# jeremy29tien/robosuite-benchmark

Hardware: AMD Instinct MI355X
Metric: SAC grad-steps/sec (batch=256, 1e6 buffer) at 1/2/4/8 GPU (higher is better)
Workload: dtype f32; 1 GPU; Lift-Panda-OSC-POSE SAC inner loop: obs 42 / act 7, batch 256, 1000000-slot HBM replay buffer (full), hidden 256x256, variant.json trainer_kwargs (lr 1e-3/5e-4, tau .005, period 5); parallelism=single GPU

## Files before the change

### robosuite_benchmark_amd/csrc/sac_fused.h

```cpp
#pragma once

constexpr int CNT_STRIDE = 32;
constexpr unsigned long long HANDOFF_TIMEOUT_TICKS = 5000000ull;

template <int SLEEP = 1>
__device__ __forceinline__ int handoff_wait(const unsigned *cnt, unsigned target, unsigned *abort_flag) {
    const unsigned long long t0 = __builtin_amdgcn_s_memrealtime();
    for (;;) {
        const unsigned v = __hip_atomic_load(cnt, __ATOMIC_RELAXED, __HIP_MEMORY_SCOPE_AGENT);
        if ((int)(v - target) >= 0) return 1;
        if (__hip_atomic_load(abort_flag, __ATOMIC_RELAXED, __HIP_MEMORY_SCOPE_AGENT) != 0u) return 0;
        if (__builtin_amdgcn_s_memrealtime() - t0 > HANDOFF_TIMEOUT_TICKS) {
            __hip_atomic_store(abort_flag, 1u, __ATOMIC_RELAXED, __HIP_MEMORY_SCOPE_AGENT);
            return 0;
        }
        __builtin_amdgcn_s_sleep(SLEEP);
    }
}

template <int SLEEP = 1>
__device__ __forceinline__ void handoff_wait_multi(int n, const unsigned *c0, unsigned t0, const unsigned *c1, unsigned t1,
                                                   const unsigned *c2, unsigned t2, unsigned *abort_flag, int *s_ok) {
    if (threadIdx.x < 64) {
        const int l = threadIdx.x;
// ... 45 lines not shown
__device__ __forceinline__ unsigned long long multi_lp_peek(int n, const unsigned *c0, const unsigned *c1, const unsigned long long *lp_tag, int NB) {
    unsigned long long w = 0ull;
    if (threadIdx.x < 64) {
        const int l = threadIdx.x;
        if (l < n) w = __hip_atomic_load(l == 0 ? c0 : c1, __ATOMIC_RELAXED, __HIP_MEMORY_SCOPE_AGENT);
        else if (l >= 16 && l < 16 + NB) w = __hip_atomic_load(lp_tag + (l - 16), __ATOMIC_RELAXED, __HIP_MEMORY_SCOPE_AGENT);
    }
    return w;
}

__device__ __forceinline__ void handoff_publish(unsigned *cnt) {
    asm volatile("s_waitcnt vmcnt(0) lgkmcnt(0)\n\ts_barrier" ::: "memory");
    if (threadIdx.x == 0) __hip_atomic_fetch_add(cnt, 1u, __ATOMIC_RELAXED, __HIP_MEMORY_SCOPE_AGENT);
}

__device__ __forceinline__ AlphaStep alpha_step_v(const Ctl *ctl, const float *part_logpi, int NB, int B, float target_entropy,
                                                  float lr, int auto_alpha, double bc1, double bc2s) {
    AlphaStep r;
    const float la = sload(&ctl->log_alpha), m0 = sload(&ctl->a_m), v0 = sload(&ctl->a_v);
    if (!auto_alpha) { r.alpha = 1.0f; r.alpha_loss = 0.0f; r.log_alpha = la; r.m = m0; r.v = v0; return r; }
    const int lane = threadIdx.x & 63;
    const float mine = part_logpi[lane < NB ? lane : 0];
    float sum = 0.f;
#pragma unroll
    for (int i = 0; i < 16; ++i)
        if (i < NB) sum += __builtin_bit_cast(float, __builtin_amdgcn_readlane(__builtin_bit_cast(int, mine), i));
    const float mean_lp = sum / (float)B + target_entropy;
    r.alpha_loss = -((la * mean_lp) + 0.0f);
    const float gr = -mean_lp;
    r.m = m0 + ADAM_1MB1 * (gr - m0);
    r.v = v0 * ADAM_B2 + ADAM_1MB2 * gr * gr;
    const float step_size = (float)((double)lr / bc1);
    const float denom = sqrtf(r.v) / (float)bc2s + 1e-8f;
    r.log_alpha = la + (-step_size * r.m) / denom;
    r.alpha = expf(r.log_alpha);
    return r;
}

template <int D>
__device__ __forceinline__ bool split_first_layer(WRing<1, D> &rq, const float *X0, int KLQ, int KS, float bq, float *zx_blk,
                                                  unsigned *cnt, unsigned target, unsigned *abort_flag, int *s_ok, int part,
                                                  f32x4 (&z)[4]) {
    const int wave = threadIdx.x >> 6, lane = threadIdx.x & 63;
    f32x4 acc[1] = {};
    gemm_ring<false, false>(rq, X0, KLQ, KS, acc);
    f32x4 zq;
#pragma unroll
    for (int i = 0; i < 4; ++i) zq[i] = acc[0][i] + bq;
    st4_sc1(zx_blk + ((part * 4 + wave) * 64 + lane) * 4, zq);
    handoff_publish(cnt);
    if (threadIdx.x == 0) *s_ok = handoff_wait(cnt, target, abort_flag);
    lds_barrier();
    if (!*s_ok) return false;
#pragma unroll
    for (int t = 0; t < 4; ++t) z[t] = ld4(zx_blk + ((wave * 4 + t) * 64 + lane) * 4);
    return true;
}

template <int PAGES>
struct ImgRegs {
    f32x4 v[PAGES];
    __device__ __forceinline__ void issue(const float *__restrict__ img, int KL) {
        const float *p = img + (threadIdx.x >> 4) * KL + 4 * (threadIdx.x & 15);
#pragma unroll
        for (int j = 0; j < PAGES; ++j) {
            v[j] = f32x4{0.f, 0.f, 0.f, 0.f};
            if (64 * j < KL) v[j] = ld4(p + 64 * j);
        }
    }
    __device__ __forceinline__ void commit(float *X, int KL, int skip_k = -1) const {
        const int row = threadIdx.x >> 4, c = threadIdx.x & 15;
        float *p = X + row * KL + 4 * c;
        const int sp = (skip_k >= 0 && ((c ^ row) >> 2) == ((skip_k >> 4) & 3)) ? (skip_k >> 6) : -1;
#pragma unroll
        for (int j = 0; j < PAGES; ++j)
            if (64 * j < KL && j != sp) st4(p + 64 * j, v[j]);
    }
};

template <int NTH, bool WIDE, int MODE = M_SAC, bool IMG = false>
__global__ __launch_bounds__(256) void k_abc(Dev d, const float *__restrict__ S, SlotLayout SL, StepArg sa) {
    kernarg_prefetch<sizeof(Dev) + 8 + sizeof(SlotLayout) + sizeof(StepArg)>();
    constexpr int SP = 4, SW = 64;
    extern __shared__ __attribute__((aligned(16))) float lds[];
    __shared__ int s_ok;
    __shared__ float s_dq[RB];
    __shared__ float s_lp[16];
    const int B = d.B, O = d.O, A = d.A, NB = d.NB;
    const int KLQ = (d.KQ + 63) & ~63;
    float *X0 = lds;
    float *X1 = X0 + RB * KLQ;
    float *XS = X1 + RB * H;
    float *red = XS + RB * SW;
    float *WL = red + FUSED_RED;
#ifndef SAC_XR_XOR
#define SAC_XR_XOR 4
#endif
    const int xq = blockIdx.x >> 3, xr = (blockIdx.x & 7) ^ SAC_XR_XOR;
    const bool isq = xr < 4;
    const int net = (xr >> 1) & 1;
    const int bi = 2 * xq + (xr & 1);
    const int part = bi & 3, rb = bi >> 2;
    const int row0 = rb * RB;
    const int wave = threadIdx.x >> 6, lane = threadIdx.x & 63, c = lane & 15, g = lane >> 4;
    const int row = threadIdx.x >> 4, a = threadIdx.x & 15, grow = row0 + row;
    const int n0 = SW * part + 16 * wave;
    unsigned *cnt_head = d.cnt, *cnt_qa = d.cnt + (size_t)2 * NB * CNT_STRIDE, *cnt_tq = d.cnt + (size_t)3 * NB * CNT_STRIDE,
             *cnt_ac = d.cnt + (size_t)4 * NB * CNT_STRIDE;
    unsigned *cnt_zx = d.cnt + (size_t)(5 * NB + 2) * CNT_STRIDE;
    unsigned long long *lp_tag = reinterpret_cast<unsigned long long *>(d.cnt + (size_t)(11 * NB + 2) * CNT_STRIDE);
    const unsigned seq = sa.seq;
    const bool own_s = isq && net == 0 && part == 0, own_n = !isq && net == 0 && part == 0;
    if ((sa.pad2 & 1u) && blockIdx.x == (4 ^ SAC_XR_XOR)) return;
    STAMP(0, 0);
    float eps = 0.f;
    f32x4 keep1[4], zkeep[4];
    float bv1[1], w3[4];
    unsigned peek = 0u;
    const bool skip_a = (MODE == M_TD3_CRITIC) && !isq && net == 0 && !(sa.pad2 & 4u);
    if (!skip_a) {
        const float *P = isq ? d.P[1 + net] : ((MODE == M_TD3_CRITIC && net == 1) ? d.P[5] : d.P[0]);
        const Layer L0 = isq ? d.LQ[0] : d.LP[0], L1 = isq ? d.LQ[1] : d.LP[1], L2 = isq ? d.LQ[2] : d.LP[2];
        const int K0 = isq ? d.KQ : d.KP;
        const float *obs = S + ((!isq && net) ? SL.off_nobs : SL.off_obs) + (size_t)row0 * O;
        RowRegs<IMG ? 1 : (WIDE ? 32 : 8)> rows;
        ImgRegs<IMG ? (WIDE ? 8 : 2) : 1> img;
        if constexpr (IMG) img.issue(S + ((!isq && net) ? SL.off_img_n : SL.off_img_sa) + (size_t)row0 * KLQ, KLQ);
        else rows.issue(K0, obs, O, O, S + SL.off_act + (size_t)row0 * A, isq ? A : 0, A, d.KP);
        WRing<4, WIDE ? 1 : RD0> r0;
        WRing<1, 8> rq;
        constexpr int PRE0 = 2;
        float bv0[4], bq = 0.f;
        if constexpr (WIDE) {
            rq.init(P + L0.offW, L0.Kp, 64 * part + 16 * wave, 16);
            rq.fill(K0 >> 4);
            bq = P[L0.offB + 64 * part + 16 * wave + c];
        } else {
            r0.init(P + L0.offW, L0.Kp, 64 * wave, 16);
            r0.fill_part(K0 >> 4, 0, PRE0);
#pragma unroll
            for (int t = 0; t < 4; ++t) bv0[t] = P[L0.offB + 64 * wave + 16 * t + c];
        }
        SB();
        WRing<1, 8> r1;
        r1.init(P + L1.offW, H, n0, 16);
        if constexpr (WIDE) r1.fill(H >> 4);
        WRing<NTH, 1> rh;
#define ABC_LATE_REQUESTS()                                                                             \
        do {                                                                                            \
            bv1[0] = P[L1.offB + n0 + c];                                                               \
            _Pragma("unroll") for (int u = 0; u < 4; ++u) w3[u] = 0.f;                                  \
            if (!isq) {                                                                                 \
                rh.init(P + L2.offW, H, 0, 16, 4 * part + wave);                                        \
                rh.fill(1);                                                                             \
            } else {                                                                                    \
                _Pragma("unroll") for (int u = 0; u < 4; ++u) w3[u] = P[L2.offW + frag_off(0, SW * part + a + 16 * u, H)]; \
            }                                                                                           \
            SB();                                                                                       \
        } while (0)
        if constexpr (WIDE) ABC_LATE_REQUESTS();
        STAMP(0, 12);
        {
            const int side0 = isq ? 0 : 1;
            const float *epp0 = side0 ? d.eps2 : d.eps1;
            if (a < A && !epp0) eps = philox_normal(d.noise_seed, (unsigned long long)sa.step_now, (unsigned)(grow * 16 + a), side0 ? 1u : 0u);
        }
        if constexpr (IMG) img.commit(X0, KLQ);
        else rows.commit(X0, KLQ, K0, O, d.KP, isq ? A : 0);
        lds_barrier();
        STAMP(0, 13);
        if constexpr (WIDE) {
            const int chain = isq ? net : 2 + net;
            if (!split_first_layer(rq, X0, KLQ, K0 >> 4, bq, d.zx + (size_t)(chain * NB + rb) * (RB * H),
                                   cnt_zx + (size_t)(chain * NB + rb) * CNT_STRIDE, 4u * seq, d.abort_flag, &s_ok, part, zkeep)) return;
#pragma unroll
            for (int t = 0; t < 4; ++t)
#pragma unroll
                for (int i = 0; i < 4; ++i) {
                    keep1[t][i] = fmaxf(zkeep[t][i], 0.f);
                    X1[lds_off(4 * g + i, 64 * wave + 16 * t + c, H)] = keep1[t][i];
                }
        } else {
            f32x4 acc[4] = {};
            gemm_straight_pf(r0, X0, KLQ, K0 >> 4, acc, r1, H >> 4, PRE0);
#pragma unroll
            for (int t = 0; t < 4; ++t)
#pragma unroll
                for (int i = 0; i < 4; ++i) zkeep[t][i] = acc[t][i] + bv0[t];
            hidden_epilogue<4>(acc, 64 * wave, 16, bv0, X1, H, keep1);
        }
        lds_barrier();
        if constexpr (!WIDE) ABC_LATE_REQUESTS();
#undef ABC_LATE_REQUESTS
        {
            f32x4 acc[1] = {};
            if (isq) gemm_ring<true>(r1, X1, H, H >> 4, acc, 0, WL + 16 * wave);
            else gemm_ring(r1, X1, H, H >> 4, acc);
            if (isq && wave == part) store_features<4, true>(keep1, 64 * wave, 16, d.QH1T + (size_t)net * H * B, B, row0);
            slice_epilogue<1, true>(acc, bv1, wave, XS, isq ? d.QH2T + (size_t)net * H * B : nullptr, n0, B, row0);
        }
        lds_barrier();
        if (!isq) {
            f32x4 acc[NTH] = {};
            gemm_ring(rh, XS, SW, 1, acc, wave);
            splitk_reduce<NTH, true>(acc, nullptr, red, d.headpart + ((size_t)(net * NB + rb) * SP + part) * (RB * 32), 32);
        } else {
            if (MODE == M_SAC && threadIdx.x == 0) peek = __hip_atomic_load(cnt_head + (size_t)rb * CNT_STRIDE, __ATOMIC_RELAXED, __HIP_MEMORY_SCOPE_AGENT);
            float s = 0.f;
#pragma unroll
            for (int u = 0; u < 4; ++u) s += XS[lds_off(row, a + 16 * u, SW)] * w3[u];
            s = group16_sum(s);
            if (a == 0) st_sc1(d.qpart2 + ((size_t)(net * NB + rb) * SP + part) * 32 + row, s);
        }
    }
    if (skip_a) {
        if (a < A && !d.eps2) eps = philox_normal(d.noise_seed, (unsigned long long)sa.step_now, (unsigned)(grow * 16 + a), 1u);
        if (WIDE && threadIdx.x == 0) __hip_atomic_fetch_add(cnt_zx + (size_t)(2 * NB + rb) * CNT_STRIDE, 1u, __ATOMIC_RELAXED, __HIP_MEMORY_SCOPE_AGENT);
    }
    STAMP(0, 1);
    if (!isq && !skip_a) handoff_publish(cnt_head + (size_t)(net * NB + rb) * CNT_STRIDE);
    if (MODE == M_TD3_CRITIC && isq) handoff_publish(cnt_qa + (size_t)rb * CNT_STRIDE);
    STAMP(0, 2);
    if (!isq && net == 0 && !skip_a) {
        if (wave == part) store_features<4, true>(keep1, 64 * wave, 16, d.PH1T, B, row0);
        f32x4 v;
#pragma unroll
        for (int i = 0; i < 4; ++i) v[i] = XS[lds_off(4 * g + i, 16 * wave + c, SW)];
        st4_sc1(d.PH2T + frag_off(n0 + c, row0 + 4 * g, B), v);
    }

    WRing<1, 8> rc;
    unsigned long long peek_c = 0ull;
    if (MODE == M_SAC || !isq) {
    const int p4 = isq ? net : 2 + net;
    const int side = isq ? 0 : 1, pass = 2 + p4;
    const float *PQ = d.P[1 + p4];
    const int KS0 = d.KQ >> 4, lo0 = (isq && !WIDE) ? KS0 - 1 : 0;
    const float *epp = side ? d.eps2 : d.eps1;
    const int am = (a < A) ? a : 0;
    const float *PH = (MODE == M_TD3_CRITIC) ? d.P[5] : d.P[0];
    const float hbm = PH[d.LP[2].offB + am], hbr = (MODE == M_SAC) ? PH[d.LP[2].offB + A + am] : 0.f;
    if (a < A && epp) eps = epp[grow * A + am];
    RowRegs<IMG ? 1 : (WIDE ? 32 : 8)> rows2;
    ImgRegs<IMG ? (WIDE ? 8 : 2) : 1> img2;
    float abat = 0.f;
    if constexpr (IMG) {
        if (!isq && net == 0) img2.issue(S + SL.off_img_n + (size_t)row0 * KLQ, KLQ);
    } else {
        if (isq) abat = S[SL.off_act + (size_t)grow * A + ((a < A) ? a : 0)];
        else rows2.issue(d.KQ, S + SL.off_nobs + (size_t)row0 * O, O, O, nullptr, 0, 0, 0);
    }
    if (threadIdx.x == 0)
        s_ok = (isq && (int)(peek - 4u * seq) >= 0) ? 1 : handoff_wait(cnt_head + (size_t)(side * NB + rb) * CNT_STRIDE, 4u * seq, d.abort_flag);
    if (isq) asm volatile("s_waitcnt vmcnt(0)" ::: "memory");
    lds_barrier();
    if (!s_ok) return;
    if (isq && threadIdx.x == 0) __hip_atomic_fetch_add(cnt_qa + (size_t)rb * CNT_STRIDE, 1u, __ATOMIC_RELAXED, __HIP_MEMORY_SCOPE_AGENT);
    STAMP(0, 3);
    float hm[SP], hr[SP];
    {
        const float *hp = d.headpart + (size_t)(side * NB + rb) * SP * (RB * 32) + row * 32;
#pragma unroll
        for (int p = 0; p < SP; ++p) {
            hm[p] = ld_sc1(hp + p * (RB * 32) + am);
            hr[p] = (MODE == M_SAC) ? ld_sc1(hp + p * (RB * 32) + A + am) : 0.f;
        }
    }
    f32x4 acc0[4];
    float bv0b[4];
    const int so0 = (WIDE && isq) ? KS0 - 1 : 0, ks0 = (WIDE && isq) ? 1 : KS0;
    WRing<4, WIDE ? RD : RD0> q0;
    WRing<1, 8> rq2;
    float bq2 = 0.f;
    if (isq) {
#pragma unroll
        for (int t = 0; t < 4; ++t) { acc0[t] = zkeep[t]; bv0b[t] = 0.f; }
    } else {
#pragma unroll
        for (int t = 0; t < 4; ++t) acc0[t] = f32x4{0.f, 0.f, 0.f, 0.f};
        if constexpr (!WIDE) {
#pragma unroll
            for (int t = 0; t < 4; ++t) bv0b[t] = PQ[d.LQ[0].offB + 64 * wave + 16 * t + c];
        } else {
#pragma unroll
            for (int t = 0; t < 4; ++t) bv0b[t] = 0.f;
        }
    }
    if constexpr (WIDE) {
        if (isq) {
            q0.init(PQ + d.LQ[0].offW, d.LQ[0].Kp, 64 * wave, 16, so0);
            q0.fill(ks0);
        } else {
            rq2.init(PQ + d.LQ[0].offW, d.LQ[0].Kp, 64 * part + 16 * wave, 16);
            rq2.fill(KS0);
            bq2 = PQ[d.LQ[0].offB + 64 * part + 16 * wave + c];
        }
    } else {
        q0.init(PQ + d.LQ[0].offW, d.LQ[0].Kp, 64 * wave, 16, so0);
        q0.fill_part(KS0, 0, RD0, lo0);
    }
    WRing<1, 8> q1;
    q1.init(PQ + d.LQ[1].offW, H, n0, 16);
    q1.fill(H >> 4);
    bv1[0] = PQ[d.LQ[1].offB + n0 + c];
#pragma unroll
    for (int u = 0; u < 4; ++u) w3[u] = PQ[d.LQ[2].offW + frag_off(0, SW * part + a + 16 * u, H)];
    SB();
    if constexpr (IMG) {
        if (!isq && net == 0) img2.commit(X0, KLQ, d.KP);
    } else {
        if (!isq) rows2.commit(X0, KLQ, d.KQ, O, 0, 0, d.KP, d.KP + 16);
    }
    float lp = 0.f, mean = 0.f, raw = 0.f, lstd = 0.f, stdv = 1.f, zz = 0.f, act = 0.f;
    USE_FROM_HERE(hm[0]);
    if (a < A) {
        mean = hm[0]; raw = hr[0];
#pragma unroll
        for (int p = 1; p < SP; ++p) { mean += hm[p]; raw += hr[p]; }
        mean += hbm; raw += hbr;
        if constexpr (MODE == M_SAC) {
            lstd = fminf(fmaxf(raw, LOG_SIG_MIN), LOG_SIG_MAX);
            stdv = expf(lstd);
            zz = __fadd_rn(mean, __fmul_rn(stdv, eps));
            act = tanhf(zz);
            const float dd = __fsub_rn(zz, mean);
            const float var = __fmul_rn(stdv, stdv);
            const float nlp = -(dd * dd) / (2.0f * var) - logf(stdv) - 0.91893853320467274178f;
            lp = nlp - logf(1.0f - act * act + TANH_EPS);
        } else {
            zz = tanhf(mean);
            act = zz + fminf(fmaxf(eps * d.td3_sigma, -d.td3_clip), d.td3_clip);
        }
    }
    {
        float *xa = X0 + lds_off(row, d.KP + a, KLQ);
        if constexpr (IMG) { if (isq) abat = *xa; }
        *xa = (a < A) ? (isq ? act - abat : act) : 0.f;
    }
    const float lsum = group16_sum(lp);
    if (own_s && a == 0) red[row] = (grow < d.Bt) ? lsum : 0.f;
    lds_barrier();
    float lsum_blk = 0.f;
    if (own_s && threadIdx.x == 0) {
        for (int i = 0; i < RB; ++i) lsum_blk += red[i];
    }
    STAMP(0, 4);
    if constexpr (WIDE) {
        if (isq) {
            gemm_ring(q0, X0, KLQ, ks0, acc0, so0);
            hidden_epilogue<4>(acc0, 64 * wave, 16, bv0b, X1, H, keep1);
        } else {
            if (!split_first_layer(rq2, X0, KLQ, KS0, bq2, d.zx + (size_t)((4 + net) * NB + rb) * (RB * H),
                                   cnt_zx + (size_t)((4 + net) * NB + rb) * CNT_STRIDE, 4u * seq, d.abort_flag, &s_ok, part, acc0)) return;
#pragma unroll
            for (int t = 0; t < 4; ++t)
#pragma unroll
                for (int i = 0; i < 4; ++i) X1[lds_off(4 * g + i, 64 * wave + 16 * t + c, H)] = fmaxf(acc0[t][i], 0.f);
        }
    } else {
        gemm_straight(q0, X0, KLQ, KS0, acc0, lo0);
        hidden_epilogue<4>(acc0, 64 * wave, 16, bv0b, X1, H, keep1);
    }
    WRing<1, 4> ra;
    if (isq) {
        SB();
        ra.init(d.PT[1 + net] + d.LQ[0].offWt, H, d.KP, 16, 4 * wave);
        ra.fill(4);
        SB();
    }
    lds_barrier();
    {
        f32x4 acc[1] = {};
        gemm_ring(q1, X1, H, H >> 4, acc);
        if (own_s) {
            if (a < A) {
                d.mu[grow * 16 + a] = mean;
                d.ls[grow * 16 + a] = lstd;
                d.z[grow * 16 + a] = zz;
                st4_sc1(d.hv4 + (size_t)(grow * 16 + a) * 4,
                        f32x4{act, lstd, eps, (raw >= LOG_SIG_MIN && raw <= LOG_SIG_MAX) ? 1.f : 0.f});
            }
            d.anew[grow * 16 + a] = act;
            if (a == 0) d.logpi[grow] = lsum;
            if (threadIdx.x == 0) { d.part_logpi[rb] = lsum_blk; tagged_publish(lp_tag + rb, lsum_blk, seq); }
        } else if (own_n) {
            d.a2[grow * 16 + a] = act;
            if (MODE == M_SAC && a == 0) { d.logpi2[grow] = lsum; st_sc1(d.logpi2p + rb * 32 + row, lsum); }
        }
        slice_epilogue<1>(acc, bv1, wave, XS, nullptr, n0, B, row0);
    }
    lds_barrier();
    {
        float s = 0.f;
#pragma unroll
        for (int u = 0; u < 4; ++u) s += XS[lds_off(row, a + 16 * u, SW)] * w3[u];
        s = group16_sum(s);
        if (a == 0) st_sc1(d.qpart2 + ((size_t)(pass * NB + rb) * SP + part) * 32 + row, s);
    }
    STAMP(0, 5);
    if (isq) {
        rc.init(d.PT[1 + net] + d.LQ[1].offWt, H, n0, 16);
        rc.fill(H >> 4);
    }
    if (isq) {
#pragma unroll
        for (int u = 0; u < 4; ++u) {
            const int off = lds_off(row, a + 16 * u, SW);
            XS[off] = (XS[off] > 0.f) ? w3[u] : 0.f;
        }
        lds_barrier();
        {
            f32x4 acc[4] = {};
            gemm_lds_rows<4, 4>(WL, 64 * wave, XS, SW, acc);
#pragma unroll
            for (int t = 0; t < 4; ++t) {
#pragma unroll
                for (int i = 0; i < 4; ++i) {
                    const int off = lds_off(4 * g + i, 64 * wave + 16 * t + c, H);
                    X1[off] = (X1[off] > 0.f) ? acc[t][i] : 0.f;
                }
            }
        }
        lds_barrier();
        {
            f32x4 acc[1] = {};
            gemm_ring(ra, X1, H, 4, acc, 4 * wave);
            splitk_reduce<1, true>(acc, nullptr, red, d.dapart + (((size_t)net * SP + part) * B + row0) * 16, 16);
        }
    }
    STAMP(0, 6);
    if (MODE == M_SAC && isq) peek_c = multi_lp_peek(2, cnt_tq + (size_t)rb * CNT_STRIDE, cnt_qa + (size_t)rb * CNT_STRIDE, lp_tag, NB);
    handoff_publish((isq ? cnt_ac : cnt_tq) + (size_t)rb * CNT_STRIDE);
    STAMP(0, 7);
    }
    if (MODE == M_TD3_CRITIC) {
        if (!isq) return;
        rc.init(d.PT[1 + net] + d.LQ[1].offWt, H, n0, 16);
        rc.fill(H >> 4);
    }

    const float invB = 1.0f / (float)d.Bt;
    const long long oB3 = d.LQ[2].offB;
    if (isq) {
        float *X2 = lds;
        const float *P = d.P[1 + net], *PT = d.PT[1 + net];
        const float *h2T = d.QH2T + (size_t)net * H * B, *h1T = d.QH1T + (size_t)net * H * B;
        const int k = threadIdx.x;
        handoff_wait_multi_lp(2, cnt_tq + (size_t)rb * CNT_STRIDE, 8u * seq, cnt_qa + (size_t)rb * CNT_STRIDE, 8u * seq, lp_tag,
                              (MODE == M_SAC) ? NB : 0, seq, d.abort_flag, &s_ok, s_lp, peek_c);
        lds_barrier();
        if (!s_ok) return;
        STAMP(0, 8);
        const float wk = P[d.LQ[2].offW + frag_off(0, k, H)];
        const float b3a = sload(d.P[3] + oB3), b3b = sload(d.P[4] + oB3), b3q = sload(P + oB3);
        float qa[SP], qb[SP], qq[SP], in_c = 0.f, in_r = 0.f, in_t = 0.f;
#pragma unroll
        for (int p = 0; p < SP; ++p) { qa[p] = 0.f; qb[p] = 0.f; qq[p] = 0.f; }
        if (threadIdx.x < RB) {
            const int r = row0 + threadIdx.x;
#pragma unroll
            for (int p = 0; p < SP; ++p) {
                qa[p] = ld_sc1(d.qpart2 + ((size_t)(4 * NB + rb) * SP + p) * 32 + threadIdx.x);
                qb[p] = ld_sc1(d.qpart2 + ((size_t)(5 * NB + rb) * SP + p) * 32 + threadIdx.x);
                qq[p] = ld_sc1(d.qpart2 + ((size_t)(net * NB + rb) * SP + p) * 32 + threadIdx.x);
            }
            if constexpr (MODE == M_SAC) in_c = ld_sc1(d.logpi2p + rb * 32 + threadIdx.x);
            in_r = S[SL.off_rew + r]; in_t = S[SL.off_term + r];
        }
        f32x4 h2v[4];
#pragma unroll
        for (int qd = 0; qd < 4; ++qd) h2v[qd] = ld4(h2T + frag_off(k, row0 + 4 * qd, B));
        f32x4 h1v[1];
        h1v[0] = ld4(h1T + frag_off(n0 + c, row0 + 4 * g, B));
        float alpha = 0.f;
        if constexpr (MODE == M_SAC)
            alpha = alpha_step_v(d.ctl, s_lp, NB, d.Bt, d.target_entropy, d.alpha_lr, d.auto_alpha, sa.bc1, sa.bc2s).alpha;
        float va = 0.f, vb = 0.f, vq = 0.f, yv = 0.f, dq = 0.f;
        if (threadIdx.x < RB) {
            va = qa[0]; vb = qb[0]; vq = qq[0];
#pragma unroll
            for (int p = 1; p < SP; ++p) { va += qa[p]; vb += qb[p]; vq += qq[p]; }
            va += b3a;
            vb += b3b;
            vq += b3q;
            const float tq = fminf(va, vb) - alpha * in_c;
            yv = bellman_target(d.reward_scale, in_r, in_t, d.discount, tq);
            dq = (row0 + (int)threadIdx.x < d.Bt) ? 2.0f * (vq - yv) * invB : 0.f;
            s_dq[threadIdx.x] = dq;
        }
        lds_barrier();
        STAMP(1, 0);
        f32x4 gv2[4];
#pragma unroll
        for (int qd = 0; qd < 4; ++qd) {
#pragma unroll
            for (int i = 0; i < 4; ++i) {
                gv2[qd][i] = (h2v[qd][i] > 0.f) ? s_dq[4 * qd + i] * wk : 0.f;
                X2[lds_off(4 * qd + i, k, H)] = gv2[qd][i];
            }
        }
        lds_barrier();
        STAMP(1, 1);
        {
            f32x4 acc[1] = {};
            gemm_ring(rc, X2, H, H >> 4, acc);
#ifdef SAC_STAMPS
            { float probe = acc[0][0]; asm volatile("" ::"v"(probe)); STAMP(1, 2); }
#endif
            if (threadIdx.x < RB && part == 0) {
// ... 123 lines not shown
```

### robosuite_benchmark_amd/csrc/sac_trainer.hip

```cpp
#include "sac_common.h"

#include <algorithm>
#include <array>
#include <cmath>
#include <cstddef>
#include <cstdlib>
#include <chrono>
#include <cstring>
#include <mutex>
#include <vector>

namespace sac {

typedef float f32x4 __attribute__((ext_vector_type(4)));

constexpr float LOG_SIG_MAX = 2.0f, LOG_SIG_MIN = -20.0f, TANH_EPS = 1e-6f;
constexpr float ADAM_B1 = 0.9f, ADAM_B2 = 0.999f, ADAM_EPS = 1e-8f;
constexpr float ADAM_1MB1 = (float)(1.0 - 0.9), ADAM_1MB2 = (float)(1.0 - 0.999);
constexpr int DIAG_TRACE_CAP = 4096;
constexpr int M_SAC = 0, M_TD3_CRITIC = 1, M_TD3_ACTOR = 2;
constexpr int RD = 4;

struct StepArg {
    long long step_now;
// ... 19 lines not shown
struct AlphaStep { float alpha, alpha_loss, log_alpha, m, v; };

struct Layer {
    int N, K, Np, Kp;
    long long offW, offB;
    long long offWt;
};

struct Net {
    float *P = nullptr, *M = nullptr, *V = nullptr, *PT = nullptr, *MT = nullptr, *VT = nullptr, *G = nullptr;
    long long nP = 0, nPT = 0;
    Layer L[3];
};

struct Dev {
    int B, Bt;
    int O, A, KP, KQ, NH, NB;
    float discount, reward_scale, tau, target_entropy, alpha_lr;
    int period, auto_alpha;
    unsigned long long noise_seed;
    Ctl *ctl;
    const float *P[6];
    int algo, sp;
    float td3_sigma, td3_clip;
    const float *PT[3];
    Layer LP[3], LQ[3];
    float *PH1T, *PH2T, *mu, *ls, *lsok, *z, *anew, *epsv, *logpi, *a2, *logpi2, *part_logpi;
    float *QH1T, *QH2T, *q;
    float *QU;
    float *y, *dq16T, *dQH2T, *dQH1T, *dheadT, *dPH2T, *dPH1T;
    float *headpart, *qpart, *dapart;
    float *qpart2, *logpi2p;
    float *hv4;
    float *zx;
    unsigned *cnt, *abort_flag;
    float *diag_first, *diag_last, *diag_trace;
    float *diag_dev;
    const float *eps1, *eps2;
};

struct DwLayer {
    const float *dYT, *XT;
    long long xt_off;
    float *P, *PT, *MT, *VT, *G;
    float *bias, *mb, *vb, *gb;
    float *TP, *Tbias;
    int N, K, ldp, ldt, nk, job0, xt_from_slot;
    float lr;
    int k_base, pad_;
};
constexpr int NDW = 12;
struct DwTable {
    const DwLayer *L;
    int job0[NDW];
    int njobs;
    const unsigned *abort;
};

#ifdef SAC_STAMPS
__device__ unsigned long long g_stamps[5 * 512 * 16];
#define STAMP(kid, i)                                                                              \
    do {                                                                                           \
        __builtin_amdgcn_sched_barrier(0);                                                         \
        if (threadIdx.x == 0 && blockIdx.x < 512) {                                                \
            g_stamps[((kid) * 512 + blockIdx.x) * 16 + (i)] = wall_clock64();                      \
        }                                                                                          \
        __builtin_amdgcn_sched_barrier(0);                                                         \
    } while (0)
#define STAMP_CLK(kid, i)                                                                          \
    do {                                                                                           \
        if (threadIdx.x == 0 && blockIdx.x < 512) g_stamps[((kid) * 512 + blockIdx.x) * 16 + (i)] = clock64(); \
    } while (0)
#else
#define STAMP(kid, i) do { } while (0)
#define STAMP_CLK(kid, i) do { } while (0)
#endif

__device__ __forceinline__ int lds_off(int row, int k, int KL) {
    return row * KL + ((((k >> 2) ^ (row & 15)) << 2) | (k & 3));
}
#define SB() __builtin_amdgcn_sched_barrier(0)
#define USE_FROM_HERE(x) asm volatile("" : "+v"(x))
__device__ __forceinline__ void lds_barrier() { asm volatile("s_waitcnt lgkmcnt(0)\n\ts_barrier" ::: "memory"); }
template <typename T>
__device__ __forceinline__ T sload(const T *p) {
    return *(const __attribute__((address_space(4))) T *)(uintptr_t)p;
}
__device__ __forceinline__ f32x4 ld4(const float *p) { return *reinterpret_cast<const f32x4 *>(p); }
#ifndef DW_ONE_GLOBAL
#define DW_ONE_GLOBAL 0
#endif
__device__ __forceinline__ f32x4 ld4g(const float *p) { return *(const __attribute__((address_space(1))) f32x4 *)(uintptr_t)p; }
__device__ __forceinline__ float ld1g(const float *p) { return *(const __attribute__((address_space(1))) float *)(uintptr_t)p; }
__device__ __forceinline__ void st1g(float *p, float v) {
    __hip_atomic_store((__attribute__((address_space(1))) float *)(uintptr_t)p, v, __ATOMIC_RELAXED, __HIP_MEMORY_SCOPE_AGENT);
}

template <int NBYTES>
__device__ __forceinline__ void kernarg_prefetch() {
    typedef const __attribute__((address_space(4))) int *kptr;
    kptr ka = (kptr)__builtin_amdgcn_kernarg_segment_ptr();
    constexpr int NL = (NBYTES + 63) / 64;
    static_assert(NL <= 16, "kernarg_prefetch: more than 16 lines");
    int x[16];
#pragma unroll
    for (int i = 0; i < 16; ++i) x[i] = ka[i < NL ? i * 16 : 0];
    asm volatile("" ::"s"(x[0]), "s"(x[1]), "s"(x[2]), "s"(x[3]), "s"(x[4]), "s"(x[5]), "s"(x[6]), "s"(x[7]), "s"(x[8]),
                 "s"(x[9]), "s"(x[10]), "s"(x[11]), "s"(x[12]), "s"(x[13]), "s"(x[14]), "s"(x[15]));
}

__device__ __forceinline__ AlphaStep alpha_step(const Ctl *ctl, const float *part_logpi, int NB, int B, float target_entropy,
                                                float lr, int auto_alpha, double bc1, double bc2s) {
    AlphaStep r;
    const float la = sload(&ctl->log_alpha), m0 = sload(&ctl->a_m), v0 = sload(&ctl->a_v);
    if (!auto_alpha) { r.alpha = 1.0f; r.alpha_loss = 0.0f; r.log_alpha = la; r.m = m0; r.v = v0; return r; }
    float sum = 0.f;
    for (int i = 0; i < NB; ++i) sum += sload(part_logpi + i);
    const float mean_lp = sum / (float)B + target_entropy;
    r.alpha_loss = -((la * mean_lp) + 0.0f);
    const float gr = -mean_lp;
    r.m = m0 + ADAM_1MB1 * (gr - m0);
    r.v = v0 * ADAM_B2 + ADAM_1MB2 * gr * gr;
    const float step_size = (float)((double)lr / bc1);
    const float denom = sqrtf(r.v) / (float)bc2s + 1e-8f;
    r.log_alpha = la + (-step_size * r.m) / denom;
    r.alpha = expf(r.log_alpha);
    return r;
}
__device__ __forceinline__ void st4(float *p, f32x4 v) { *reinterpret_cast<f32x4 *>(p) = v; }

template <int NT, int D = RD>
struct WRing {
    f32x4 b[D][NT];
    const float *wp[NT];
    __device__ __forceinline__ void init(const float *W, int ldw, int n_base, int n_stride, int s_off = 0) {
        const int lane = threadIdx.x & 63;
#pragma unroll
        for (int t = 0; t < NT; ++t)
            wp[t] = W + ((size_t)((n_base + t * n_stride) >> 4) * (ldw >> 4) + s_off) * 256 + 4 * lane;
    }
    __device__ __forceinline__ void fill_part(int KS, int u0, int u1, int lo = 0) {
#pragma unroll
        for (int u = 0; u < D; ++u)
            if (u >= u0 && u < u1 && u < KS && u >= lo) {
#pragma unroll
                for (int t = 0; t < NT; ++t) b[u][t] = ld4(wp[t] + 256 * u);
            }
    }
    __device__ __forceinline__ void fill(int KS) {
#pragma unroll
        for (int u = 0; u < D; ++u)
            if (u < KS) {
#pragma unroll
                for (int t = 0; t < NT; ++t) b[u][t] = ld4(wp[t] + 256 * u);
            }
    }
};

template <bool STAGED = false, bool ALT = true, int NT, int D>
__device__ __forceinline__ void gemm_ring(WRing<NT, D> &R, const float *X, int KL, int KS, f32x4 (&acc)[NT],
                                          int s_off = 0, float *stage = nullptr) {
    const int lane = threadIdx.x & 63;
    const int r = lane & 15, g = lane >> 4;
    const float *xrow = X + r * KL;
    f32x4 a_cur = ld4(xrow + 4 * ((4 * s_off + g) ^ r));
    f32x4 acc_odd = {0.f, 0.f, 0.f, 0.f};
    for (int S0 = 0; S0 < KS; S0 += D) {
#pragma unroll
        for (int u = 0; u < D; ++u) {
            const int S = S0 + u;
            if (S < KS) {
                const int Sn = (S + 1 < KS) ? S + 1 : S;
                const f32x4 a_nxt = ld4(xrow + 4 * ((4 * (Sn + s_off) + g) ^ r));
                if constexpr (STAGED) {
#pragma unroll
                    for (int t = 0; t < NT; ++t)
#pragma unroll
                        for (int i = 0; i < 4; ++i) stage[(16 * S + 4 * g + i) * WLD + 16 * t + r] = R.b[u][t][i];
                }
                SB();
#pragma unroll
                for (int i = 0; i < 4; ++i) {
                    if constexpr (NT == 1 && ALT) {
                        if (i & 1) acc_odd = __builtin_amdgcn_mfma_f32_16x16x4f32(a_cur[i], R.b[u][0][i], acc_odd, 0, 0, 0);
                        else acc[0] = __builtin_amdgcn_mfma_f32_16x16x4f32(a_cur[i], R.b[u][0][i], acc[0], 0, 0, 0);
                    } else {
#pragma unroll
                        for (int t = 0; t < NT; ++t)
                            acc[t] = __builtin_amdgcn_mfma_f32_16x16x4f32(a_cur[i], R.b[u][t][i], acc[t], 0, 0, 0);
                    }
                }
                SB();
                if (S + D < KS) {
#pragma unroll
                    for (int t = 0; t < NT; ++t) R.b[u][t] = ld4(R.wp[t] + 256 * (S + D));
                }
                SB();
                a_cur = a_nxt;
            }
        }
    }
    if constexpr (NT == 1 && ALT) acc[0] += acc_odd;
}

template <int NT, int KS>
__device__ __forceinline__ void gemm_lds_rows(const float *WL, int col0, const float *X, int KL, f32x4 (&acc)[NT]) {
    const int lane = threadIdx.x & 63;
    const int r = lane & 15, g = lane >> 4;
    const float *xrow = X + r * KL;
    f32x4 a[KS], bf[KS][NT];
#pragma unroll
    for (int S = 0; S < KS; ++S) {
        a[S] = ld4(xrow + 4 * ((4 * S + g) ^ r));
#pragma unroll
        for (int t = 0; t < NT; ++t) bf[S][t] = ld4(WL + (col0 + 16 * t + r) * WLD + 16 * S + 4 * g);
    }
#pragma unroll
    for (int S = 0; S < KS; ++S)
#pragma unroll
        for (int i = 0; i < 4; ++i)
#pragma unroll
            for (int t = 0; t < NT; ++t) acc[t] = __builtin_amdgcn_mfma_f32_16x16x4f32(a[S][i], bf[S][t][i], acc[t], 0, 0, 0);
}

template <int NT, int D>
__device__ __forceinline__ void gemm_straight(WRing<NT, D> &R, const float *X, int KL, int KS, f32x4 (&acc)[NT],
                                              int lo = 0) {
    const int lane = threadIdx.x & 63;
    const int r = lane & 15, g = lane >> 4;
    const float *xrow = X + r * KL;
#pragma unroll
    for (int u = 0; u < D; ++u) {
        if (u >= lo && u < KS) {
            const f32x4 a = ld4(xrow + 4 * ((4 * u + g) ^ r));
#pragma unroll
            for (int i = 0; i < 4; ++i) {
#pragma unroll
                for (int t = 0; t < NT; ++t)
                    acc[t] = __builtin_amdgcn_mfma_f32_16x16x4f32(a[i], R.b[u][t][i], acc[t], 0, 0, 0);
            }
        }
    }
}
template <int NT, int D, int NT1, int D1>
__device__ __forceinline__ void gemm_straight_pf(WRing<NT, D> &R, const float *X, int KL, int KS, f32x4 (&acc)[NT],
                                                 WRing<NT1, D1> &R1, int KS1, int pre = D) {
    const int lane = threadIdx.x & 63;
    const int r = lane & 15, g = lane >> 4;
    const float *xrow = X + r * KL;
    constexpr int Q1 = (D1 + 3) / 4;
#pragma unroll
    for (int u = 0; u < D; ++u) {
        if (u + pre < D) {
            SB();
            R.fill_part(KS, u + pre, u + pre + 1);
            SB();
        }
        if (u < KS) {
            const f32x4 a = ld4(xrow + 4 * ((4 * u + g) ^ r));
#ifdef SAC_STAMPS
            if (u < 4) { float probe = R.b[u][NT - 1][3]; asm volatile("" ::"v"(probe)); STAMP(0, 5 + u); }
#endif
#pragma unroll
            for (int i = 0; i < 4; ++i) {
#pragma unroll
                for (int t = 0; t < NT; ++t)
                    acc[t] = __builtin_amdgcn_mfma_f32_16x16x4f32(a[i], R.b[u][t][i], acc[t], 0, 0, 0);
            }
        }
        if (u < 4) {
            SB();
            R1.fill_part(KS1, u * Q1, (u + 1) * Q1);
            SB();
        }
    }
}

__device__ __forceinline__ void st_sc1(float *p, float v) { __hip_atomic_store(p, v, __ATOMIC_RELAXED, __HIP_MEMORY_SCOPE_AGENT); }
__device__ __forceinline__ float ld_sc1(const float *p) { return __hip_atomic_load(p, __ATOMIC_RELAXED, __HIP_MEMORY_SCOPE_AGENT); }
__device__ __forceinline__ void st4_sc1(float *p, f32x4 v) {
    asm volatile("global_store_dwordx4 %0, %1, off sc1\n\ts_nop 1" ::"v"(p), "v"(v) : "memory");
}

template <int NTT, bool SC1 = false>
__device__ __forceinline__ void splitk_reduce(const f32x4 (&acc)[NTT], const float *__restrict__ bias, float *red,
                                              float *out, int ldo) {
    const int wave = threadIdx.x >> 6, lane = threadIdx.x & 63;
#pragma unroll
    for (int t = 0; t < NTT; ++t) st4(red + ((wave * NTT + t) * 64 + lane) * 4, acc[t]);
    lds_barrier();
    if constexpr (SC1) {
        for (int e = threadIdx.x; e < NTT * 64; e += 256) {
            const int t = e >> 6, row = (e >> 2) & 15, c0 = 4 * (e & 3);
            f32x4 s4;
#pragma unroll
            for (int j = 0; j < 4; ++j) {
                const int l = (row >> 2) * 16 + c0 + j, i = row & 3;
                float s = 0.f;
#pragma unroll
                for (int w = 0; w < 4; ++w) s += red[((w * NTT + t) * 64 + l) * 4 + i];
                s4[j] = s;
            }
            st4_sc1(out + row * ldo + 16 * t + c0, s4);
        }
    } else {
        for (int e = threadIdx.x; e < NTT * 256; e += 256) {
// ... 32 lines not shown
    const float u1 = ((float)(c0 >> 8) + 0.5f) * (1.0f / 16777216.0f);
    const float u2 = ((float)(c1 >> 8) + 0.5f) * (1.0f / 16777216.0f);
    return sqrtf(-2.0f * logf(u1)) * cosf(6.28318530717958647692f * u2);
}

__device__ __forceinline__ float bellman_target(float reward_scale, float r, float term, float discount, float tq) {
    return fmaf(reward_scale, r, __fmul_rn(__fmul_rn(1.0f - term, discount), tq));
}
__device__ __forceinline__ float polyak_mix(float t, float p, float tau) { return fmaf(t, 1.0f - tau, __fmul_rn(p, tau)); }
__device__ __forceinline__ f32x4 polyak_mix4(f32x4 t, f32x4 p, float tau) {
    f32x4 o;
#pragma unroll
    for (int i = 0; i < 4; ++i) o[i] = polyak_mix(t[i], p[i], tau);
    return o;
}
__device__ __forceinline__ float actor_da(float da1, float dq1, float da2, float dq2) { return fmaf(da1, dq1, __fmul_rn(da2, dq2)); }
__device__ __forceinline__ float actor_dz(float da, float om, float alpha_invB, float act) {
    return fmaf(da, om, __fmul_rn(alpha_invB, __fdiv_rn(__fmul_rn(__fmul_rn(2.0f, act), om), __fadd_rn(om, TANH_EPS))));
}
__device__ __forceinline__ float actor_dls(float dz, float stdv, float eps, float alpha_invB, float ok) {
    return __fmul_rn(fmaf(__fmul_rn(dz, stdv), eps, -alpha_invB), ok);
}

template <int ROWS_MAXE>
struct RowRegs {
    float v[ROWS_MAXE];
    __device__ __forceinline__ void issue(int Kfill, const float *__restrict__ s0, int n0, int ld0,
                                          const float *__restrict__ s1, int n1, int ld1, int c1) {
        const int nper = Kfill >> 4;
        const int row = threadIdx.x >> 4, p = threadIdx.x & 15;
        const float *r0 = s0 + row * ld0;
        const float *r1 = (n1 > 0 ? s1 + row * ld1 : r0) - (n1 > 0 ? c1 : 0);
#pragma unroll
        for (int i = 0; i < ROWS_MAXE; ++i) {
            v[i] = 0.f;
            if (i < nper) {
                const int k = p + 16 * i;
                const float *src = (k < n0) ? r0 + k : ((k >= c1 && k < c1 + n1) ? r1 + k : r0);
                v[i] = *src;
            }
        }
    }
    __device__ __forceinline__ void commit(float *X, int KL, int Kfill, int n0, int c1, int n1, int skip_lo = 0,
                                           int skip_hi = 0) const {
        const int nper = Kfill >> 4;
        const int row = threadIdx.x >> 4, p = threadIdx.x & 15;
#pragma unroll
        for (int i = 0; i < ROWS_MAXE; ++i)
            if (i < nper) {
                const int k = p + 16 * i;
                const bool valid = (k < n0) || (k >= c1 && k < c1 + n1);
                if (k < skip_lo || k >= skip_hi) X[lds_off(row, k, KL)] = valid ? v[i] : 0.f;
            }
    }
};

template <int NT>
__device__ __forceinline__ void hidden_epilogue(const f32x4 (&acc)[NT], int n_base, int n_stride,
                                                const float (&bv)[NT], float *Xn, int KL, f32x4 (&keep)[NT]) {
    const int lane = threadIdx.x & 63, c = lane & 15, g = lane >> 4;
#pragma unroll
    for (int t = 0; t < NT; ++t) {
        const int n = n_base + t * n_stride + c;
#pragma unroll
        for (int i = 0; i < 4; ++i) {
            keep[t][i] = fmaxf(acc[t][i] + bv[t], 0.f);
            Xn[lds_off(4 * g + i, n, KL)] = keep[t][i];
        }
    }
}
template <int NT, bool SC1 = false>
__device__ __forceinline__ void store_features(const f32x4 (&v)[NT], int n_base, int n_stride, float *outT, int B, int row0) {
    const int lane = threadIdx.x & 63, c = lane & 15, g = lane >> 4;
#pragma unroll
    for (int t = 0; t < NT; ++t) {
        float *p = outT + frag_off(n_base + t * n_stride + c, row0 + 4 * g, B);
        if constexpr (SC1) st4_sc1(p, v[t]);
        else st4(p, v[t]);
    }
}

constexpr int ring_depth(int ntw) { return ntw == 1 ? 8 : 4; }

template <int NTW, bool SC1 = false>
__device__ __forceinline__ void slice_epilogue(const f32x4 (&acc)[NTW], const float (&bv)[NTW], int wave, float *XS,
                                               float *outT, int n_first, int B, int row0) {
    const int lane = threadIdx.x & 63, c = lane & 15, g = lane >> 4;
#pragma unroll
    for (int t = 0; t < NTW; ++t) {
        f32x4 v;
#pragma unroll
        for (int i = 0; i < 4; ++i) {
            v[i] = fmaxf(acc[t][i] + bv[t], 0.f);
            XS[lds_off(4 * g + i, 16 * (NTW * wave + t) + c, 64 * NTW)] = v[i];
        }
        if (outT) {
            float *p = outT + frag_off(n_first + 16 * t + c, row0 + 4 * g, B);
            if constexpr (SC1) st4_sc1(p, v);
            else st4(p, v);
        }
    }
}

template <int NTH, bool WIDE, int SP, int MODE = M_SAC>
__device__ __forceinline__ void fwd_a_body(const Dev &d, const float *__restrict__ S, const SlotLayout &SL, int aux) {
    constexpr int NTW = 4 / SP, SW = 64 * NTW;
    extern __shared__ __attribute__((aligned(16))) float lds[];
    const int B = d.B, O = d.O, A = d.A, NB = d.NB;
    const int KLmax = (d.KQ + 63) & ~63;
    float *X0 = lds;
    float *X1 = X0 + RB * KLmax;
    float *XS = X1 + RB * H;
    float *red = XS + RB * SW;
    const int xq = blockIdx.x >> 3, xr = blockIdx.x & 7;
    const bool is_pi = xr < 4;
    const int b = is_pi ? 4 * xq + xr : 2 * xq + (xr & 1);
    const int part = b % SP, rb = (b / SP) % NB;
    const int sq = is_pi ? (b / SP) / NB : ((xr - 4) >> 1);
    const int row0 = rb * RB;
    const int wave = threadIdx.x >> 6, lane = threadIdx.x & 63, c = lane & 15;
    const int row = threadIdx.x >> 4, p16 = threadIdx.x & 15;
    if constexpr (MODE != M_SAC) { if (is_pi && sq == 0 && !aux) return; }
    const float *P = is_pi ? ((MODE != M_SAC && sq == 1) ? d.P[5] : d.P[0]) : d.P[1 + sq];
    const Layer L0 = is_pi ? d.LP[0] : d.LQ[0], L1 = is_pi ? d.LP[1] : d.LQ[1], L2 = is_pi ? d.LP[2] : d.LQ[2];
    const int K0 = is_pi ? d.KP : d.KQ, KL0 = (K0 + 63) & ~63;
    const int n0 = SW * part + 16 * NTW * wave;
    const float *obs = S + ((is_pi && sq) ? SL.off_nobs : SL.off_obs) + (size_t)row0 * O;

    STAMP(0, 0);
    RowRegs<WIDE ? 32 : 8> rows;
    rows.issue(K0, obs, O, O, S + SL.off_act + (size_t)row0 * A, is_pi ? 0 : A, A, d.KP);
    WRing<4, WIDE ? RD : RD0> r0;
    r0.init(P + L0.offW, L0.Kp, 64 * wave, 16);
    constexpr int PRE0 = 2;
    if constexpr (WIDE) r0.fill(K0 >> 4);
    else r0.fill_part(K0 >> 4, 0, PRE0);
    float bv0[4];
#pragma unroll
    for (int t = 0; t < 4; ++t) bv0[t] = P[L0.offB + 64 * wave + 16 * t + c];
    SB();
    WRing<NTW, ring_depth(NTW)> r1;
    r1.init(P + L1.offW, H, n0, 16);
    if constexpr (WIDE) r1.fill(H >> 4);
    float bv1[NTW];
    WRing<NTH, NTW> rh;
    float w3[4 * NTW];
#define FWD_A_LATE_REQUESTS()                                                                          \
    do {                                                                                               \
        _Pragma("unroll") for (int t = 0; t < NTW; ++t) bv1[t] = P[L1.offB + n0 + 16 * t + c];         \
        _Pragma("unroll") for (int u = 0; u < 4 * NTW; ++u) w3[u] = 0.f;                               \
        if (is_pi) {                                                                                   \
            rh.init(P + L2.offW, H, 0, 16, 4 * NTW * part + NTW * wave);                               \
            rh.fill(NTW);                                                                              \
        } else {                                                                                       \
            _Pragma("unroll") for (int u = 0; u < 4 * NTW; ++u) w3[u] = P[L2.offW + frag_off(0, SW * part + p16 + 16 * u, H)]; \
        }                                                                                              \
        SB();                                                                                          \
    } while (0)
    if constexpr (WIDE) FWD_A_LATE_REQUESTS();
    rows.commit(X0, KL0, K0, O, d.KP, is_pi ? 0 : A);
    lds_barrier();
    STAMP(0, 1);
    f32x4 keep1[4], zkeep[4];
    {
        f32x4 acc[4] = {};
        if constexpr (WIDE) gemm_ring(r0, X0, KL0, K0 >> 4, acc);
        else {
            gemm_straight_pf(r0, X0, KL0, K0 >> 4, acc, r1, H >> 4, PRE0);
        }
#pragma unroll
        for (int t = 0; t < 4; ++t)
#pragma unroll
            for (int i = 0; i < 4; ++i) zkeep[t][i] = acc[t][i] + bv0[t];
        hidden_epilogue<4>(acc, 64 * wave, 16, bv0, X1, H, keep1);
    }
    lds_barrier();
    STAMP(0, 2);
// ... 2457 lines not shown
```

Baseline: 39010 grad-steps/s.

## Fuse actor-tail relu mask into epilogue, interleave Q partial with MFMA, drop barriers

In the actor Q-backprop tail, the relu-masked w3 gradient is now written to a separate LDS buffer (G2, aliasing X0) inside slice_epilogue, so the separate masking pass and one block barrier go away. The Q-partial dot product and its shuffle reduction are interleaved step by step between the MFMA groups of the tail GEMM, and the mask for X1 uses register-held keep1 values instead of re-reading LDS. The barrier before the final ring GEMM becomes a wave-local lgkmcnt wait, justified by each wave only reading its own columns. The rc weight-ring init is hoisted earlier. The risk is LDS aliasing of X0 and subtle races if the own-column assumption is wrong.

```diff
diff --git a/robosuite_benchmark_amd/csrc/sac_fused.h b/robosuite_benchmark_amd/csrc/sac_fused.h
--- a/robosuite_benchmark_amd/csrc/sac_fused.h
+++ b/robosuite_benchmark_amd/csrc/sac_fused.h
@@ -151,6 +151,8 @@
 __global__ __launch_bounds__(256) void k_abc(Dev d, const float *__restrict__ S, SlotLayout SL, StepArg sa) {
     kernarg_prefetch<sizeof(Dev) + 8 + sizeof(SlotLayout) + sizeof(StepArg)>();
     constexpr int SP = 4, SW = 64;
+    constexpr int NTW = 1;
+    constexpr int TAIL_NT = 4, TAIL_KS = 4;
     extern __shared__ __attribute__((aligned(16))) float lds[];
     __shared__ int s_ok;
     __shared__ float s_dq[RB];
@@ -158,6 +160,7 @@
     const int B = d.B, O = d.O, A = d.A, NB = d.NB;
     const int KLQ = (d.KQ + 63) & ~63;
     float *X0 = lds;
+    float *G2 = X0;
     float *X1 = X0 + RB * KLQ;
     float *XS = X1 + RB * H;
     float *red = XS + RB * SW;
@@ -266,12 +269,12 @@
             if (isq) gemm_ring<true>(r1, X1, H, H >> 4, acc, 0, WL + 16 * wave);
             else gemm_ring(r1, X1, H, H >> 4, acc);
             if (isq && wave == part) store_features<4, true>(keep1, 64 * wave, 16, d.QH1T + (size_t)net * H * B, B, row0);
-            slice_epilogue<1, true>(acc, bv1, wave, XS, isq ? d.QH2T + (size_t)net * H * B : nullptr, n0, B, row0);
+            slice_epilogue<NTW, true>(acc, bv1, wave, XS, isq ? d.QH2T + (size_t)net * H * B : nullptr, n0, B, row0);
         }
         lds_barrier();
         if (!isq) {
             f32x4 acc[NTH] = {};
-            gemm_ring(rh, XS, SW, 1, acc, wave);
+            gemm_ring(rh, XS, SW, NTW, acc, NTW * wave);
             splitk_reduce<NTH, true>(acc, nullptr, red, d.headpart + ((size_t)(net * NB + rb) * SP + part) * (RB * 32), 32);
         } else {
             if (MODE == M_SAC && threadIdx.x == 0) peek = __hip_atomic_load(cnt_head + (size_t)rb * CNT_STRIDE, __ATOMIC_RELAXED, __HIP_MEMORY_SCOPE_AGENT);
@@ -430,11 +433,12 @@
         gemm_straight(q0, X0, KLQ, KS0, acc0, lo0);
         hidden_epilogue<4>(acc0, 64 * wave, 16, bv0b, X1, H, keep1);
     }
-    WRing<1, 4> ra;
+    WRing<1, TAIL_KS> ra;
     if (isq) {
         SB();
-        ra.init(d.PT[1 + net] + d.LQ[0].offWt, H, d.KP, 16, 4 * wave);
-        ra.fill(4);
+        ra.init(d.PT[1 + net] + d.LQ[0].offWt, H, d.KP, 16, TAIL_KS * wave);
+        ra.fill(TAIL_KS);
+        rc.init(d.PT[1 + net] + d.LQ[1].offWt, H, n0, 16);
         SB();
     }
     lds_barrier();
@@ -456,44 +460,66 @@
             d.a2[grow * 16 + a] = act;
             if (MODE == M_SAC && a == 0) { d.logpi2[grow] = lsum; st_sc1(d.logpi2p + rb * 32 + row, lsum); }
         }
-        slice_epilogue<1>(acc, bv1, wave, XS, nullptr, n0, B, row0);
+        static_assert(NTW == 1 && SW == 64, "G2 takes the first [16][64] floats of X0 (KLQ >= 64)");
+        if (isq) {
+            const float w3own = (wave == 0) ? w3[0] : ((wave == 1) ? w3[1] : ((wave == 2) ? w3[2] : w3[3]));
+            slice_epilogue<NTW, false, true>(acc, bv1, wave, XS, nullptr, n0, B, row0, G2, w3own);
+        } else {
+            slice_epilogue<NTW>(acc, bv1, wave, XS, nullptr, n0, B, row0);
+        }
     }
     lds_barrier();
-    {
-        float s = 0.f;
-#pragma unroll
-        for (int u = 0; u < 4; ++u) s += XS[lds_off(row, a + 16 * u, SW)] * w3[u];
-        s = group16_sum(s);
-        if (a == 0) st_sc1(d.qpart2 + ((size_t)(pass * NB + rb) * SP + part) * 32 + row, s);
+    float qx[4], qs = 0.f;
+    auto q_partial_read = [&]() {
+#pragma unroll
+        for (int u = 0; u < 4; ++u) qx[u] = XS[lds_off(row, a + 16 * u, SW)];
+    };
+    auto q_partial_dot = [&]() {
+#pragma unroll
+        for (int u = 0; u < 4; ++u) qs += qx[u] * w3[u];
+    };
+    float *qdst = d.qpart2 + ((size_t)(pass * NB + rb) * SP + part) * 32 + row;
+    USE_FROM_HERE(qdst);
+    auto q_partial_store = [&]() {
+        if (a == 0) st1g(qdst, qs);
+    };
+    if (!isq) {
+        q_partial_read();
+        q_partial_dot();
+        qs = group16_sum(qs);
+        q_partial_store();
     }
     STAMP(0, 5);
     if (isq) {
-        rc.init(d.PT[1 + net] + d.LQ[1].offWt, H, n0, 16);
         rc.fill(H >> 4);
-    }
-    if (isq) {
-#pragma unroll
-        for (int u = 0; u < 4; ++u) {
-            const int off = lds_off(row, a + 16 * u, SW);
-            XS[off] = (XS[off] > 0.f) ? w3[u] : 0.f;
-        }
-        lds_barrier();
         {
-            f32x4 acc[4] = {};
-            gemm_lds_rows<4, 4>(WL, 64 * wave, XS, SW, acc);
-#pragma unroll
-            for (int t = 0; t < 4; ++t) {
+            float qt = 0.f;
+            auto side = [&](auto G) {
+                constexpr int k = decltype(G)::value;
+                if constexpr (k == 3) q_partial_read();
+                else if constexpr (k == 6) { q_partial_dot(); qt = __shfl_xor(qs, 1); }
+                else if constexpr (k == 8) { qs += qt; qt = __shfl_xor(qs, 2); }
+                else if constexpr (k == 10) { qs += qt; qt = __shfl_xor(qs, 4); }
+                else if constexpr (k == 12) { qs += qt; qt = __shfl_xor(qs, 8); }
+                else if constexpr (k == 14) { qs += qt; q_partial_store(); }
+            };
+            f32x4 acc[TAIL_NT] = {};
+            gemm_lds_rows_side<TAIL_NT, SW / 16>(WL, 16 * TAIL_NT * wave, G2, SW, acc, side);
+#pragma unroll
+            for (int t = 0; t < TAIL_NT; ++t) {
 #pragma unroll
                 for (int i = 0; i < 4; ++i) {
-                    const int off = lds_off(4 * g + i, 64 * wave + 16 * t + c, H);
-                    X1[off] = (X1[off] > 0.f) ? acc[t][i] : 0.f;
+                    static_assert(TAIL_NT == 4, "keep1[t][i] is element (4 g + i, 64 wave + 16 t + c) of X1");
+                    X1[lds_off(4 * g + i, 16 * TAIL_NT * wave + 16 * t + c, H)] = (keep1[t][i] > 0.f) ? acc[t][i] : 0.f;
                 }
             }
         }
-        lds_barrier();
+        static_assert(wave_reads_own_columns(16 * TAIL_NT, TAIL_KS, TAIL_KS) && 4 * 16 * TAIL_NT == H,
+                      "actor tail: a wave contracts X1 columns of another wave");
+        lds_wave_fence();
         {
             f32x4 acc[1] = {};
-            gemm_ring(ra, X1, H, 4, acc, 4 * wave);
+            gemm_ring(ra, X1, H, TAIL_KS, acc, TAIL_KS * wave);
             splitk_reduce<1, true>(acc, nullptr, red, d.dapart + (((size_t)net * SP + part) * B + row0) * 16, 16);
         }
     }
diff --git a/robosuite_benchmark_amd/csrc/sac_trainer.hip b/robosuite_benchmark_amd/csrc/sac_trainer.hip
--- a/robosuite_benchmark_amd/csrc/sac_trainer.hip
+++ b/robosuite_benchmark_amd/csrc/sac_trainer.hip
@@ -125,6 +125,10 @@
 #define SB() __builtin_amdgcn_sched_barrier(0)
 #define USE_FROM_HERE(x) asm volatile("" : "+v"(x))
 __device__ __forceinline__ void lds_barrier() { asm volatile("s_waitcnt lgkmcnt(0)\n\ts_barrier" ::: "memory"); }
+__device__ __forceinline__ void lds_wave_fence() { asm volatile("s_waitcnt lgkmcnt(0)" ::: "memory"); }
+constexpr bool wave_reads_own_columns(int cols_per_wave, int ks, int s_off_per_wave) {
+    return cols_per_wave == 16 * ks && s_off_per_wave == ks;
+}
 template <typename T>
 __device__ __forceinline__ T sload(const T *p) {
     return *(const __attribute__((address_space(4))) T *)(uintptr_t)p;
@@ -265,6 +269,34 @@
 #pragma unroll
             for (int t = 0; t < NT; ++t) acc[t] = __builtin_amdgcn_mfma_f32_16x16x4f32(a[S][i], bf[S][t][i], acc[t], 0, 0, 0);
 }
+template <int G>
+struct Step { static constexpr int value = G; };
+template <int NT, int KS, int G, typename Side>
+__device__ __forceinline__ void lds_rows_groups(const f32x4 (&a)[KS], const f32x4 (&bf)[KS][NT], f32x4 (&acc)[NT], Side &side) {
+    if constexpr (G < 4 * KS) {
+        constexpr int S = G >> 2, i = G & 3;
+#pragma unroll
+        for (int t = 0; t < NT; ++t) acc[t] = __builtin_amdgcn_mfma_f32_16x16x4f32(a[S][i], bf[S][t][i], acc[t], 0, 0, 0);
+        SB();
+        side(Step<G>{});
+        SB();
+        lds_rows_groups<NT, KS, G + 1>(a, bf, acc, side);
+    }
+}
+template <int NT, int KS, typename Side>
+__device__ __forceinline__ void gemm_lds_rows_side(const float *WL, int col0, const float *X, int KL, f32x4 (&acc)[NT], Side &side) {
+    const int lane = threadIdx.x & 63;
+    const int r = lane & 15, g = lane >> 4;
+    const float *xrow = X + r * KL;
+    f32x4 a[KS], bf[KS][NT];
+#pragma unroll
+    for (int S = 0; S < KS; ++S) {
+        a[S] = ld4(xrow + 4 * ((4 * S + g) ^ r));
+#pragma unroll
+        for (int t = 0; t < NT; ++t) bf[S][t] = ld4(WL + (col0 + 16 * t + r) * WLD + 16 * S + 4 * g);
+    }
+    lds_rows_groups<NT, KS, 0>(a, bf, acc, side);
+}
 
 template <int NT, int D>
 __device__ __forceinline__ void gemm_straight(WRing<NT, D> &R, const float *X, int KL, int KS, f32x4 (&acc)[NT],
@@ -463,9 +495,11 @@
 
 constexpr int ring_depth(int ntw) { return ntw == 1 ? 8 : 4; }
 
-template <int NTW, bool SC1 = false>
+template <int NTW, bool SC1 = false, bool MASKED = false>
 __device__ __forceinline__ void slice_epilogue(const f32x4 (&acc)[NTW], const float (&bv)[NTW], int wave, float *XS,
-                                               float *outT, int n_first, int B, int row0) {
+                                               float *outT, int n_first, int B, int row0, float *G2 = nullptr,
+                                               float wown = 0.f) {
+    static_assert(!MASKED || NTW == 1, "slice_epilogue<MASKED>: one own weight per lane = one tile per wave");
     const int lane = threadIdx.x & 63, c = lane & 15, g = lane >> 4;
 #pragma unroll
     for (int t = 0; t < NTW; ++t) {
@@ -473,7 +507,9 @@
 #pragma unroll
         for (int i = 0; i < 4; ++i) {
             v[i] = fmaxf(acc[t][i] + bv[t], 0.f);
-            XS[lds_off(4 * g + i, 16 * (NTW * wave + t) + c, 64 * NTW)] = v[i];
+            const int off = lds_off(4 * g + i, 16 * (NTW * wave + t) + c, 64 * NTW);
+            XS[off] = v[i];
+            if constexpr (MASKED) G2[off] = (v[i] > 0.f) ? wown : 0.f;
         }
         if (outT) {
             float *p = outT + frag_off(n_first + 16 * t + c, row0 + 4 * g, B);
```

New measurement: 39710 grad-steps/s (median of 6 runs). 1.8% higher.
